# kanster/moped

Measured on AMD Instinct MI355X. Metric: detections/sec (frames/s) 640x480 ~3k SIFT vs N models, higher is better.
Workload: dtype f32

## Files before the change

include/moped_hip.h:

```cpp
#ifndef MOPED_HIP_H
#define MOPED_HIP_H

#include <stddef.h>
#include <stdint.h>

#ifdef __cplusplus
extern "C" {
#endif

#define MH_DESC_DIM 128
#define MH_MAX_BATCH 32
#define MH_MAX_IMAGES 8
#define MH_MAX_MODELS 8192
#define MH_OK 0
#define MH_ERR_ARG (-1)
#define MH_ERR_HIP (-2)
#define MH_ERR_CAPACITY (-3)
#define MH_ERR_NODEVICE (-4)

typedef struct mh_ctx mh_ctx;


int mh_create(int device, mh_ctx** out);
void mh_destroy(mh_ctx* ctx);
// ... 40 lines not shown
int mh_screen_values(mh_ctx* ctx, const float* q_host, int Q, int n_rows, float* out_host, float* dmax, float* spread,
                     int shape );
uint16_t mh_screen_record_value(float top, float thr);
void mh_screen_record_bounds(uint16_t value_bits, uint32_t row0, float tau, float spread, int N, float dmax, float* lo,
                             float* hi);
float mh_screen_pack_value(float v, uint32_t id, int bits);
float mh_screen_pack_pert(float qq, float dmax, int bits);
void mh_screen_sample_bounds(uint16_t value_bits, float tau, float pert, float dmax, float* lo, float* hi);
void mh_screen_launch_plan(int Q, int q_expected, int N, int32_t out[8]);
int mh_match_incomplete(mh_ctx* ctx, uint32_t* count, int reset);
int mh_screen_sample_values(mh_ctx* ctx, const float* q_host, int Q, const int32_t* row0_host, float* out_host);
int mh_match_query_candidates(mh_ctx* ctx, int Q, uint32_t* out);

int mh_match_local_dev(mh_ctx* ctx, const float* qn_dev, const float* qnorm_dev, int Q,
                       int32_t* idx1_dev, float* d1_dev, float* d2_dev);
int mh_match_merge_dev(mh_ctx* ctx, const int32_t* idx1_s_dev, const float* d1_s_dev,
                       const float* d2_s_dev, int n_shards, int Q,
                       int32_t* idx1_dev, float* d1_dev, float* d2_dev);
int mh_normalize_dev(mh_ctx* ctx, float* q_dev, float* qnorm_dev, int Q);


int mh_meanshift(mh_ctx* ctx, const float* pts_host, int n, int dim, float radius,
                 float merge, int min_pts, int max_iter, int32_t* label,
                 int32_t* order, int32_t* n_clusters);
int mh_meanshift_batch(mh_ctx* ctx, const float* pts_host, const int32_t* off, int n_problems,
                       int dim, float radius, float merge, int min_pts, int max_iter,
                       int32_t* label, int32_t* order, int32_t* n_clusters);


typedef struct {
// ... 304 lines not shown
```

moped_amd/capi.py:

```python
from __future__ import annotations

import ctypes as C
import os

import numpy as np

_HERE = os.path.dirname(os.path.abspath(__file__))
LIB_PATH = os.environ.get("MH_LIB_PATH") or os.path.join(_HERE, "libmoped_hip.so")

MH_OK = 0


class MhError(RuntimeError):
    pass


class mh_corr(C.Structure):
    _fields_ = [("u", C.c_float), ("v", C.c_float), ("x", C.c_float), ("y", C.c_float), ("z", C.c_float)]


class mh_cam(C.Structure):
    _fields_ = [("K", C.c_float * 4), ("cam", C.c_float * 7)]


# ... 50 lines not shown
        super().__init__(cutoff, min_pts, use3d_filter, sigma2d, sigma3d, linkage_type)


def default_linkage_params():
    return mh_linkage_params(0.1, 7, 2, -1.0, -1.0, 1)


class mh_depth_rules(C.Structure):
    _fields_ = [("patch_size", C.c_int32), ("feature_density", C.c_float), ("match_density", C.c_float),
                ("ratio_table", C.c_void_p), ("n_models", C.c_int32), ("maximum_depth", C.c_float),
                ("default_depth", C.c_float), ("cauchy_scale", C.c_float)]


EXPORTS = [
    "mh_create", "mh_destroy", "mh_last_error", "mh_set_stream", "mh_synchronize", "mh_reserve",
    "mh_db_upload", "mh_db_size", "mh_normalize", "mh_match", "mh_normalize_match", "mh_match_local_dev",
    "mh_match_merge_dev", "mh_normalize_dev", "mh_meanshift", "mh_meanshift_batch", "mh_pose_ransac", "mh_pose_ransac_depth",
    "mh_frame_set_depth", "mh_project_test",
    "mh_filter", "mh_frame_default_params", "mh_frame_enqueue", "mh_frame_set_depth_image", "mh_frame_enqueue_match_local",
    "mh_frame_enqueue_rest", "mh_frame_fetch", "mh_frame_result_dev", "mh_enable_timing", "mh_timing",
    "mh_frame_set_cluster_linkage", "mh_cluster_linkage", "mh_frame_set_depth_image_host",
    "mh_depth_fill", "mh_depth_fill_status", "mh_depth_fill_host",
    "mh_frame_enqueue_rest_batch", "mh_frame_enqueue_rest_frames", "mh_frame_fetch_slot", "mh_frame_result_copy_slots_dev",
    "mh_frame_set_depth_rules", "mh_frame_fetch_matches", "mh_frame_enqueue_rest_strided", "mh_frame_result_copy_dev",
    "mh_sift_extract", "mh_sift_extract_dev", "mh_frame_enqueue_image", "mh_frame_enqueue_image_batch", "mh_frame_features_dev", "mh_frame_keypoints",
    "mh_models_create", "mh_models_destroy", "mh_models_last_error", "mh_models_add_xml",
    "mh_models_add_xml_buffer", "mh_models_count", "mh_models_rows", "mh_models_name", "mh_models_range",
    "mh_models_desc", "mh_models_xyz", "mh_models_save", "mh_models_load", "mh_db_upload_models",
    "mh_db_splice", "mh_db_reserve", "mh_db_adopt", "mh_db_generation", "mh_db_model_rows", "mh_db_splice_models",
    "mh_db_debug_fetch", "mh_depth_rules_debug_fetch", "mh_db_debug_screen", "mh_db_debug_route", "mh_db_edit_ms",
    "mh_db_upload_raw", "mh_db_share", "mh_match_stats", "mh_match_set_mode", "mh_match_launches", "mh_pose_set_split", "mh_frame_fetch_match_points", "mh_screen_margin", "mh_frame_counters", "mh_match_timing", "mh_frame_set_images", "mh_filter_images",
# ... 43 lines not shown
    L.mh_last_error.restype = C.c_char_p
    L.mh_set_stream.argtypes = [vp, vp]
    L.mh_synchronize.argtypes = [vp]
    L.mh_reserve.argtypes = [vp, i32, i32, i32]
    L.mh_reserve_batch.argtypes = [vp, i32, i32, i32, i32]
    if hasattr(L, "mh_lane_create"):
        L.mh_lane_create.argtypes = [i32, i32, i32, i32, C.POINTER(vp)]
        L.mh_lane_destroy.argtypes = [vp]
        L.mh_set_lane.argtypes = [vp, vp]
    L.mh_db_upload.argtypes = [vp, vp, vp, vp, i32, i32, C.c_int32]
    L.mh_db_size.argtypes = [vp, C.POINTER(i32), C.POINTER(i32)]
    L.mh_normalize.argtypes = [vp, vp, i32]
    L.mh_match.argtypes = [vp, vp, i32, f32, vp, vp, vp, vp]
    L.mh_normalize_match.argtypes = [vp, vp, i32, f32, vp, vp, vp, vp]
    L.mh_match_local_dev.argtypes = [vp, vp, vp, i32, vp, vp, vp]
    L.mh_match_merge_dev.argtypes = [vp, vp, vp, vp, i32, i32, vp, vp, vp]
    L.mh_normalize_dev.argtypes = [vp, vp, vp, i32]
    L.mh_meanshift.argtypes = [vp, vp, i32, i32, f32, f32, i32, i32, vp, vp, C.POINTER(C.c_int32)]
    L.mh_meanshift_batch.argtypes = [vp, vp, vp, i32, i32, f32, f32, i32, i32, vp, vp, vp]
    L.mh_pose_ransac.argtypes = [vp, vp, vp, i32, C.POINTER(mh_cam), C.POINTER(mh_pose_params),
                                 C.c_uint64, vp, C.POINTER(C.c_int32)]
    L.mh_pose_ransac_depth.argtypes = [vp, vp, vp, vp, i32, C.POINTER(mh_cam), C.POINTER(mh_pose_params), i32, f32,
                                       C.c_uint64, vp, C.POINTER(C.c_int32)]
    L.mh_frame_set_depth.argtypes = [vp, vp, i32, f32]
    L.mh_project_test.argtypes = [vp, vp, vp, i32, C.POINTER(mh_cam), f32, vp, vp, C.POINTER(C.c_int32)]
    L.mh_filter.argtypes = [vp, vp, vp, i32, vp, vp, i32, C.POINTER(mh_cam), i32, f32, f32,
                            vp, vp, vp, vp, vp, C.POINTER(C.c_int32)]
    L.mh_frame_default_params.argtypes = [C.POINTER(mh_frame_params)]
    L.mh_frame_default_params.restype = None
    L.mh_frame_enqueue.argtypes = [vp, vp, vp, i32, C.POINTER(mh_cam), C.POINTER(mh_frame_params), C.c_uint64]
# ... 1172 lines not shown
        counts = np.zeros(4, np.int32)
        self._ck(self.L.mh_frame_fetch(self.h, _ptr(objs), max_objects, C.byref(n), _ptr(counts)), "mh_frame_fetch")
        return objs[:min(n.value, max_objects)].copy(), counts

    def frame_result_dev(self):
        p = C.c_void_p()
        b = C.c_int64(0)
        self._ck(self.L.mh_frame_result_dev(self.h, C.byref(p), C.byref(b)), "mh_frame_result_dev")
        return p.value, b.value

    def match_local_dev(self, qn_ptr, qnorm_ptr, Q, idx_ptr, d1_ptr, d2_ptr):
        self._ck(self.L.mh_match_local_dev(self.h, C.c_void_p(qn_ptr), C.c_void_p(qnorm_ptr), Q,
                                           C.c_void_p(idx_ptr), C.c_void_p(d1_ptr), C.c_void_p(d2_ptr)),
                 "mh_match_local_dev")

    def match_merge_dev(self, idx_s_ptr, d1_s_ptr, d2_s_ptr, n_shards, Q, idx_ptr, d1_ptr, d2_ptr):
        self._ck(self.L.mh_match_merge_dev(self.h, C.c_void_p(idx_s_ptr), C.c_void_p(d1_s_ptr),
                                           C.c_void_p(d2_s_ptr), n_shards, Q, C.c_void_p(idx_ptr),
                                           C.c_void_p(d1_ptr), C.c_void_p(d2_ptr)), "mh_match_merge_dev")

    def normalize_dev(self, q_ptr, qnorm_ptr, Q):
        self._ck(self.L.mh_normalize_dev(self.h, C.c_void_p(q_ptr), C.c_void_p(qnorm_ptr), Q), "mh_normalize_dev")


class ModelSet:

    def __init__(self, desc_type: str = "SIFT", _handle=None):
        self.L = load()
        if _handle is None:
            h = C.c_void_p()
# ... 84 lines not shown
```

moped_amd/csrc/api.hip:

```cpp
#include <algorithm>
#include <cmath>
#include <cstring>
#include <new>
#include <vector>

#include "context.h"
#include "steps.h"

using namespace mh;

namespace mh {

int use_stream(mh_ctx* ctx) {
  if (!ctx->held.empty()) db_poll_held(ctx, false);
  if (ctx->stream) return MH_OK;
  if (!ctx->own_stream) MH_HIP(ctx, hipStreamCreateWithFlags(&ctx->own_stream, hipStreamNonBlocking));
  ctx->stream = ctx->own_stream;
  return MH_OK;
}

int ensure_scratch(mh_ctx* ctx, size_t bytes) {
  if (bytes > ctx->scratch.cap) MH_HIP(ctx, ctx->scratch.ensure(bytes + bytes / 4 + 4096, ctx->stream));
  return MH_OK;
}
// ... 70 lines not shown
              const int32_t* q_count, int q_expected) {
  if (Q <= 0) return MH_OK;
  int rc = ensure_match_scratch(ctx, Q);
  if (rc) return rc;
  const int qe = (q_expected > 0 && q_expected < Q) ? q_expected : Q;
  const int screen_mode = ctx->match_mode >= 2 ? 0 : ctx->match_mode;
  const int kernel_pin = ctx->match_mode >= 2 ? ctx->match_mode - 2 : -1;
  if (ctx->sdb.usable && ctx->sbuf.q_pad >= screen_q_pad(Q) && screen_wanted(qe, ctx->N, screen_mode)) {
    ctx->sbuf.ev = nullptr;
    if (ctx->timing && ctx->ev_made) {
      ctx->sbuf.ev = ctx->mev[ctx->mev_next];
      ctx->mev_next = (ctx->mev_next + 1) % mh_ctx::MEV_SETS;
      ++ctx->mev_used;
    }
    ctx->sbuf.big = ctx->lane_stream;
    ctx->sbuf.ev_in = ctx->lane_in;
    ctx->sbuf.ev_out = ctx->lane_out;
    launch_match_screen(qn, qnorm, Q, ctx->db_desc, ctx->db_norm, ctx->N, ctx->rmap, ctx->sdb, ctx->sbuf, idx1, d1,
                        d2, ctx->stream, q_count, q_expected);
    ++ctx->match_launches[2];
  } else {
    const int k = launch_match(qn, qnorm, Q, ctx->db_desc, ctx->db_norm, ctx->N, ctx->rmap, ctx->match_scratch,
                               ctx->match_pack, idx1, d1, d2, ctx->stream, q_count, q_expected, kernel_pin);
    if (k >= 0) ++ctx->match_launches[k];
  }
  return MH_OK;
}

int ensure_frame_buffers(mh_ctx* ctx, int Q) {
  if (Q <= ctx->max_q) return MH_OK;
// ... 16 lines not shown
extern "C" {

int mh_create(int device, mh_ctx** out) {
  if (!out) return MH_ERR_ARG;
  *out = nullptr;
  int count = 0;
  if (hipGetDeviceCount(&count) != hipSuccess || count <= 0 || device < 0 || device >= count)
    return MH_ERR_NODEVICE;
  hipDeviceProp_t prop;
  if (hipGetDeviceProperties(&prop, device) != hipSuccess) return MH_ERR_NODEVICE;
  if (std::strncmp(prop.gcnArchName, "gfx950", 6) != 0) return MH_ERR_NODEVICE;
  if (hipSetDevice(device) != hipSuccess) return MH_ERR_HIP;
  mh_ctx* ctx = new (std::nothrow) mh_ctx;
  if (!ctx) return MH_ERR_HIP;
  ctx->device = device;
  ctx->stream = nullptr;
  *out = ctx;
  return MH_OK;
}

void mh_free_frame_state(mh_ctx* ctx);
void mh_free_sift_state(mh_ctx* ctx);
void mh_free_undistort_state(mh_ctx* ctx);

void mh_destroy(mh_ctx* ctx) {
  if (!ctx) return;
  hipSetDevice(ctx->device);
  if (ctx->stream) hipStreamSynchronize(ctx->stream);
  mh_free_frame_state(ctx);
  mh_free_sift_state(ctx);
// ... 273 lines not shown
}

int mh_match_local_dev(mh_ctx* ctx, const float* qn_dev, const float* qnorm_dev, int Q,
                       int32_t* idx1_dev, float* d1_dev, float* d2_dev) {
  if (!ctx || Q < 0 || (Q > 0 && (!qn_dev || !qnorm_dev || !idx1_dev || !d1_dev || !d2_dev)))
    return MH_ERR_ARG;
  if (Q == 0) return MH_OK;
  MH_HIP(ctx, hipSetDevice(ctx->device));
  if (int rc_stream = mh::use_stream(ctx)) return rc_stream;
  int rc = ctx_match(ctx, qn_dev, qnorm_dev, Q, idx1_dev, d1_dev, d2_dev);
  if (rc) return rc;
  MH_HIP(ctx, hipGetLastError());
  return MH_OK;
}

int mh_match_merge_dev(mh_ctx* ctx, const int32_t* idx1_s_dev, const float* d1_s_dev,
                       const float* d2_s_dev, int n_shards, int Q, int32_t* idx1_dev,
                       float* d1_dev, float* d2_dev) {
  if (!ctx || Q < 0 || n_shards < 0) return MH_ERR_ARG;
  if (Q == 0) return MH_OK;
  MH_HIP(ctx, hipSetDevice(ctx->device));
  if (int rc_stream = mh::use_stream(ctx)) return rc_stream;
  launch_match_merge(idx1_s_dev, d1_s_dev, d2_s_dev, n_shards, Q, (size_t)Q, idx1_dev, d1_dev, d2_dev,
                     ctx->stream);
  MH_HIP(ctx, hipGetLastError());
  return MH_OK;
}

static int match_host(mh_ctx* ctx, const float* q_host, float* normalized_out, int Q, float ratio, int32_t* nn_idx,
                      int32_t* nn_raw, float* d1, float* d2) {
// ... 280 lines not shown
```

moped_amd/csrc/context.h:

```cpp
#pragma once
#include <cmath>
#include <cstring>
#include <memory>
#include <mutex>
#include <string>
#include <vector>

#include "common.h"
#include "devbuf.h"
#include "screen.h"
#include "steps.h"

struct DbStore;

struct DbPool {
  std::mutex mu;
  size_t cap_rows = 0;
  int max_models = 0;
  DbStore* spare = nullptr;
  ~DbPool();
};

struct DbStore {
  int device = 0;
// ... 59 lines not shown
  st->screen.zero_idx = (int32_t)h[4];
  std::memcpy(&st->screen.zero_d1, &h[5], 4);
  std::memcpy(&st->screen.zero_d2, &h[6], 4);
  st->screen.usable = h[2] == 0 && x_max < 60000.f;
}

struct mh_lane {
  int device = 0;
  std::vector<hipStream_t> streams;
  unsigned next = 0;
  int reserve = 0, low_priority = 0;
};

struct mh_ctx {
  int device = 0;
  hipStream_t own_stream = nullptr;
  hipStream_t stream = nullptr;
  std::string err;

  std::shared_ptr<DbStore> store;
  int N = 0, n_models = 0;
  int32_t index_base = 0;
  mh::RowMap rmap;
  float* db_desc = nullptr;
  float* db_norm = nullptr;
  float* db_xyz = nullptr;
  int32_t* db_model = nullptr;
  mh::ScreenDb sdb;
  mh::ScreenBufs sbuf;
  struct ScreenOwn {
// ... 192 lines not shown
```

moped_amd/csrc/match_screen.hip:

```cpp
#include <hip/hip_fp16.h>

#include <algorithm>
#include <cstdlib>

#include "common.h"
#include "screen.h"

MH_TRACE_TU()

namespace mh {

namespace {

typedef _Float16 half8 __attribute__((ext_vector_type(8)));
typedef float v16f __attribute__((ext_vector_type(16)));
#define MH_AS1 __attribute__((address_space(1)))
#define MH_AS3 __attribute__((address_space(3)))

constexpr int SC_QPAD = 3 * 1024;
constexpr int SC_TILE = 128;
constexpr int SC_TILE_BYTES = SC_TILE * DIM * 2;
constexpr bool SC_SHAPE16_LARGE = true;
constexpr int SC_NW_LARGE = 8;
__host__ __device__ constexpr int sc_recbuf(int nw) { return nw >= 8 ? 112 : 40; }
// ... 963 lines not shown
  const float lose = better ? a.b1 : d;
  a.b2 = fminf(a.b2, lose);
  a.b1 = better ? d : a.b1;
  a.i1 = better ? row : a.i1;
}
__device__ __forceinline__ void merge(Best& a, float ob1, float ob2, int oi1) {
  const bool take_o = (ob1 < a.b1) || (ob1 == a.b1 && (unsigned)oi1 < (unsigned)a.i1);
  const float lose1 = take_o ? a.b1 : ob1;
  const float s2 = fminf(a.b2, ob2);
  a.b2 = fminf(lose1, s2);
  a.b1 = take_o ? ob1 : a.b1;
  a.i1 = take_o ? oi1 : a.i1;
}

constexpr int RS_WAVES = 4;
constexpr int RS_MAXC = 1024;
constexpr int RS_STAGE = 8;
static_assert(RS_STAGE * DIM * 4 <= RS_MAXC * 4 && RS_STAGE % 2 == 0 && RS_STAGE <= 32, "staged rows live in the candidate list's LDS");

__device__ __forceinline__ float exact_dist(const float* __restrict__ q_lds, const float* __restrict__ row, float nq, float dn) {
  float s = 0.f;
  const float4* r4 = reinterpret_cast<const float4*>(row);
#pragma unroll 2
  for (int c = 0; c < DIM / 16; ++c) {
    const float4 x0 = r4[4 * c], x1 = r4[4 * c + 1], x2 = r4[4 * c + 2], x3 = r4[4 * c + 3];
    const float4 y0 = *reinterpret_cast<const float4*>(q_lds + 16 * c), y1 = *reinterpret_cast<const float4*>(q_lds + 16 * c + 4);
    const float4 y2 = *reinterpret_cast<const float4*>(q_lds + 16 * c + 8), y3 = *reinterpret_cast<const float4*>(q_lds + 16 * c + 12);
    s = fmaf(y0.x, x0.x, s); s = fmaf(y0.y, x0.y, s); s = fmaf(y0.z, x0.z, s); s = fmaf(y0.w, x0.w, s);
    s = fmaf(y1.x, x1.x, s); s = fmaf(y1.y, x1.y, s); s = fmaf(y1.z, x1.z, s); s = fmaf(y1.w, x1.w, s);
    s = fmaf(y2.x, x2.x, s); s = fmaf(y2.y, x2.y, s); s = fmaf(y2.z, x2.z, s); s = fmaf(y2.w, x2.w, s);
// ... 18 lines not shown
  for (int s = 0; s < 4; ++s) a[s] = ap[4 * s];
  const int crow = (g < 2 ? row0x : row0y) + 16 * (g & 1);
  const float4 c = *reinterpret_cast<const float4*>(dneg + (size_t)(crow >> 7) * SC_DD + (crow & 127));
  v4f acc = {c.x, c.y, c.z, c.w};
#pragma unroll
  for (int s = 0; s < 4; ++s) {
    const float4 y0 = *reinterpret_cast<const float4*>(q_lds + 32 * s + 8 * g), y1 = *reinterpret_cast<const float4*>(q_lds + 32 * s + 8 * g + 4);
    half8 b;
    b[0] = (_Float16)y0.x; b[1] = (_Float16)y0.y; b[2] = (_Float16)y0.z; b[3] = (_Float16)y0.w;
    b[4] = (_Float16)y1.x; b[5] = (_Float16)y1.y; b[6] = (_Float16)y1.z; b[7] = (_Float16)y1.w;
    acc = __builtin_amdgcn_mfma_f32_16x16x32_f16(a[s], b, acc, 0, 0, 0);
  }
  return acc;
}

__global__ __launch_bounds__(64 * RS_WAVES) __attribute__((amdgpu_waves_per_eu(8, 8))) void rescore_kernel(
    const float* __restrict__ qn, const float* __restrict__ qnorm, const uint8_t* __restrict__ qbad, int Q,
    const int32_t* __restrict__ q_count, const float* __restrict__ db, const float* __restrict__ dnorm, int N,
    RowMap rmap, uint2* __restrict__ recs, int n_slots, int32_t* __restrict__ ovf_cnt, uint2* __restrict__ ovf,
    int ovf_cap, float dmax, const float* __restrict__ tau, float spread, int32_t* __restrict__ idx1, float* __restrict__ d1, float* __restrict__ d2,
    unsigned int* __restrict__ stats, int32_t zero_idx, float zero_d1, float zero_d2, SampleGeom g,
    const unsigned int* __restrict__ inc, unsigned int* __restrict__ inc_count, const _Float16* __restrict__ dbh,
    const float* __restrict__ dneg) {
  MH_TRACE_SCOPE(mh::TK_PASS_C);
  __shared__ __attribute__((aligned(16))) float q_s[RS_WAVES][DIM];
  __shared__ __attribute__((aligned(16))) int cand_s[RS_WAVES][RS_MAXC];
  __shared__ int ncand_s[RS_WAVES];
  __shared__ int samp_s[RS_WAVES][SC_SA_SLOTS];
  __shared__ int nsamp_s[RS_WAVES];
  const int lane = threadIdx.x & 63;
  const int wave = __builtin_amdgcn_readfirstlane(threadIdx.x >> 6);
  const int q = blockIdx.x * RS_WAVES + wave;
  if (q >= Q) return;
  constexpr int RS_ITERS = (SC_SLOT_PITCH + SCREEN_OVF_CAP + 63) / 64;
  uint2* mine = recs + (size_t)q * SC_SLOT_PITCH;
  const int n_own = n_slots + g.sa_slots;
  auto slot_at = [&](int j) -> uint2& { return mine[j < n_slots ? j : SC_SLOTS_MAX + (j - n_slots)]; };
  uint2 recv[RS_ITERS];
#pragma unroll
  for (int it = 0; it < RS_ITERS; ++it) {
    const int j = it * 64 + lane;
    recv[it] = j < n_own ? slot_at(j) : make_uint2(0u, 0u);
  }
  const int Qe = q_count ? min(Q, *q_count) : Q;
  const int bad = qbad[q];
  const float nq = qnorm[q];
  const float tau_q = tau[q];
  const int n_ovf = ovf_cnt[q];
  const unsigned incw = inc ? inc[q] : 0u;
  const float2 qv = reinterpret_cast<const float2*>(qn + (size_t)q * DIM)[lane];
  asm volatile("" ::"v"(bad), "v"(nq), "v"(tau_q), "v"(n_ovf), "v"(incw), "v"(qv.x), "v"(qv.y), "s"(Qe));
  if (q >= Qe) {
    if (lane == 0) {
      idx1[q] = -1;
      d1[q] = __builtin_inff();
      d2[q] = __builtin_inff();
    }
    return;
  }
  if (bad == 2) {
    if (lane == 0) {
      idx1[q] = -1;
      d1[q] = __builtin_inff();
      d2[q] = __builtin_inff();
    }
    return;
  }
  if (bad == 3) {
    if (lane == 0) {
      idx1[q] = zero_idx >= 0 ? row_to_global(rmap, zero_idx) : -1;
      d1[q] = zero_d1;
      d2[q] = zero_d2;
      if (stats) stats[3 * q + 2] += 1u;
    }
    return;
  }
  if (lane == 0) {
    ncand_s[wave] = 0;
    nsamp_s[wave] = 0;
  }
  q_s[wave][2 * lane] = qv.x;
  q_s[wave][2 * lane + 1] = qv.y;
  bool brute = n_ovf > ovf_cap || bad == 1;
  int n_cand = 0;
  if (!brute) {
    float l1 = -__builtin_inff(), l2 = -__builtin_inff();
    const float pert = screen_pack_pert(nq, dmax, g.pack_bits);
    auto bounds = [tau_q, spread, N, dmax, pert](uint2 rec, float& lo, float& hi) {
      if (rec.x & SC_REC_SAMPLE) screen_sample_bounds((unsigned short)(rec.y >> 16), tau_q, pert, dmax, lo, hi);
      else screen_record_bounds((unsigned short)(rec.y >> 16), rec.x & 0x3FFFFFFFu, tau_q, spread, N, dmax, lo, hi);
    };
#pragma unroll
    for (int it = 0; it < RS_ITERS; ++it) {
      const int j = it * 64 + lane;
      uint2 rec = recv[it];
      if (j < n_own) {
        if (rec.y) slot_at(j) = make_uint2(0u, 0u);
// ... 15 lines not shown
      l1 = fmaxf(l1, o1);
    }
    const float keep_from = l2 - screen_margin(nq, dmax);
#pragma unroll
    for (int it = 0; it < RS_ITERS; ++it) {
      const uint2 rec = recv[it];
      unsigned bits = rec.y & 0xFFFFu;
      if (bits) {
        float lo, hi;
        bounds(rec, lo, hi);
        if (hi < keep_from) bits = 0;
      }
      const int hi_stride = (rec.x & 0x80000000u) ? 16 : 8;
      const int row0 = (int)(rec.x & 0x3FFFFFFFu);
      if (bits && (rec.x & SC_REC_SAMPLE)) {
        const int w = atomicAdd(&nsamp_s[wave], 1);
        if (w < SC_SA_SLOTS) samp_s[wave][w] = row0;
        bits = 0;
      }
      while (bits) {
        const int r = __builtin_ctz(bits);
        bits &= bits - 1;
        const int w = atomicAdd(&ncand_s[wave], 1);
        if (w < RS_MAXC) cand_s[wave][w] = row0 + (r & 3) + hi_stride * (r >> 2);
      }
    }
    wave_lds_sync();
    const int n_samp = min(nsamp_s[wave], SC_SA_SLOTS), n_pad_rows = (N + SC_TILE - 1) / SC_TILE * SC_TILE;
    for (int p = 0; p < n_samp; p += 2) {
      const bool pair = p + 1 < n_samp;
      const int rx = samp_s[wave][p], ry = samp_s[wave][pair ? p + 1 : p];
      if (rx + 19 >= n_pad_rows || ry + 19 >= n_pad_rows) continue;
      const v4f w = sample_pair_values(q_s[wave], dbh, dneg, rx, ry, lane);
      const int grp = lane >> 4;
      if ((lane & 15) == 0 && (grp < 2 || pair)) {
        const int base = (grp < 2 ? rx : ry) + 16 * (grp & 1);
#pragma unroll
        for (int r = 0; r < 4; ++r)
          if (w[r] > tau_q) {
            const int at = atomicAdd(&ncand_s[wave], 1);
            if (at < RS_MAXC) cand_s[wave][at] = base + r;
          }
      }
    }
    if (n_samp) wave_lds_sync();
    n_cand = ncand_s[wave];
    if (n_cand > RS_MAXC) brute = true;
  } else if (n_ovf > ovf_cap) {
    for (int j = lane; j < n_own; j += 64) slot_at(j) = make_uint2(0u, 0u);
  }
  if (n_ovf && lane == 0) ovf_cnt[q] = 0;
  wave_lds_sync();

  Best best = {__builtin_inff(), __builtin_inff(), -1};
  const int n_rows = brute ? N : n_cand;
  if (!brute && n_cand <= 64) {
    const int my_row = lane < n_cand ? cand_s[wave][lane] : -1;
    const bool my_ok = my_row >= 0 && my_row < N;
    const float my_dn = my_ok ? dnorm[my_row] : 0.f;
    wave_lds_sync();
    float4* stage = reinterpret_cast<float4*>(cand_s[wave]);
    const int n_st = min(n_cand, RS_STAGE);
    const int half = lane >> 5, c = lane & 31;
    float4 v[RS_STAGE / 2];
#pragma unroll
    for (int i = 0; i < RS_STAGE / 2; ++i) {
      const int r = 2 * i + half;
      const int row_r = __shfl(my_row, r);
      v[i] = make_float4(0.f, 0.f, 0.f, 0.f);
      if (r < n_st && row_r >= 0 && row_r < N) v[i] = reinterpret_cast<const float4*>(db + (size_t)row_r * DIM)[c];
    }
#pragma unroll
    for (int i = 0; i < RS_STAGE / 2; ++i) {
      const int r = 2 * i + half;
      if (r < n_st) stage[r * 32 + (c ^ r)] = v[i];
    }
    wave_lds_sync();
    if (lane < n_st) {
      if (my_ok) {
        float sdot = 0.f;
        const float4* qs4 = reinterpret_cast<const float4*>(q_s[wave]);
#pragma unroll 8
        for (int k = 0; k < 32; ++k) {
          const float4 x = stage[lane * 32 + (k ^ lane)], y = qs4[k];
          sdot = fmaf(y.x, x.x, sdot); sdot = fmaf(y.y, x.y, sdot); sdot = fmaf(y.z, x.z, sdot); sdot = fmaf(y.w, x.w, sdot);
        }
        take(best, fmaxf(fmaf(-2.f, sdot, nq + my_dn), 0.f), my_row);
      }
    } else if (my_ok) {
      take(best, exact_dist(q_s[wave], db + (size_t)my_row * DIM, nq, my_dn), my_row);
    }
  } else {
    for (int k = lane; k < n_rows; k += 64) {
      const int row = brute ? k : cand_s[wave][k];
      if (row >= 0 && row < N) take(best, exact_dist(q_s[wave], db + (size_t)row * DIM, nq, dnorm[row]), row);
    }
  }
  if (incw && !brute) {
    for (unsigned sm = incw & 0x0FFFFFFFu; sm; sm &= sm - 1) {
      const int split = __builtin_ctz(sm);
      const int sel0 = split * g.tiles_base + min(split, g.tiles_rem);
      const int sel1 = min(sel0 + g.tiles_base + (split < g.tiles_rem ? 1 : 0), g.n_sel);
      for (int k = sel0 * SC_TILE + lane; k < sel1 * SC_TILE; k += 64) {
        const int row = (g.tile_first + (k >> 7) * g.tile_stride) * SC_TILE + (k & 127);
        if (((incw >> (28 + ((k & 15) >> 2))) & 1u) && row < N)
          take(best, exact_dist(q_s[wave], db + (size_t)row * DIM, nq, dnorm[row]), row);
      }
    }
    if (lane == 0 && inc_count) atomicAdd(inc_count, 1u);
  }
#pragma unroll
  for (int d = 1; d < 64; d <<= 1) {
    const float ob1 = __shfl_xor(best.b1, d), ob2 = __shfl_xor(best.b2, d);
    const int oi1 = __shfl_xor(best.i1, d);
    if (oi1 >= 0) merge(best, ob1, ob2, oi1);
  }
  if (lane == 0) {
    idx1[q] = best.i1 >= 0 ? row_to_global(rmap, best.i1) : -1;
    d1[q] = best.b1;
    d2[q] = best.b2;
    if (stats) {
      stats[3 * q] += (unsigned)n_cand;
      stats[3 * q + 1] += brute ? 1u : 0u;
      stats[3 * q + 2] += 1u;
    }
  }
}

__global__ __launch_bounds__(64) void screen_values_kernel(const _Float16* __restrict__ qh, const _Float16* __restrict__ dbh,
                                                           const float* __restrict__ dneg, int n_rows, float* __restrict__ out,
                                                           int shape16) {
  const int lane = threadIdx.x, half = lane >> 5, l32 = lane & 31;
  const int q0 = blockIdx.x * 32, r0 = blockIdx.y * 32;
  if (shape16) {
    const int quarter = lane >> 4, l16 = lane & 15;
#pragma unroll
    for (int ti = 0; ti < 2; ++ti)
#pragma unroll
      for (int tj = 0; tj < 2; ++tj) {
        v4f acc;
#pragma unroll
        for (int r = 0; r < 4; ++r) {
// ... 253 lines not shown
  a.n_sel = p.n_sel_b;
  a.tile_first = 0;
  a.tile_stride = 1;
  a.skip_first = p.onesweep ? p.tile_first : 0;
  a.skip_stride = p.onesweep ? p.stride : 0;
  a.n_splits = p.Sb;
  a.tiles_base = p.n_sel_b / p.Sb;
  a.tiles_rem = p.n_sel_b % p.Sb;
  a.sub_cap = p.sub_cap;
  hipLaunchKernelGGL((screen16_kernel<1, NQB>), dim3(nqb * p.Sb), dim3(512), SC_LDS16_BYTES, s, a);
  if (ev) hipEventRecord(ev[4], s);
  *n_slots_out = 4 * p.Sb * a.sub_cap;
  *geom_out = g;
}

struct ShapeChoice {
  int nqb_sel;
  bool passes16;
};
ShapeChoice choose_shape(int qe, int n_tiles) {
  static const int nqb_pin = exp_int("MH_SCREEN_NQB", 0);
  int nqb_sel = qe > 640 ? 2 : 1;
  if (qe >= 2048 && (long)n_tiles * ((qe + 1023) / 1024) >= 16L * 256) nqb_sel = 4;
  if (nqb_pin >= 1 && nqb_pin <= 4) nqb_sel = nqb_pin;
  static const int shape_pin = exp_int("MH_SCREEN_SHAPE", 0);
  const bool shape16 = shape_pin == 2 || (shape_pin == 0 && SC_SHAPE16_LARGE);
  const bool p16 = shape16 && ((nqb_sel == 4 && (shape_pin == 2 || (qe + 1023) / 1024 >= 12)) || (nqb_sel == 2 && shape_pin == 2));
  return {nqb_sel, p16};
}

// ... 68 lines not shown
  SampleGeom geom = {0, 0, 0, 1, 0, 0, 0};
  static const int nw_pin = exp_int("MH_SCREEN_NW", 0);
  const int nw_sel = nw_pin == 4 || nw_pin == 8 ? nw_pin : (nqb_sel == 4 ? SC_NW_LARGE : 8);
  if (shape.passes16 && nqb_sel == 4) launch_passes16<4>(a, Q, qe, n_tiles, sample, blocks_a, blocks_b, &n_slots, &geom, sb.inc, sb.ev, sbig);
  else if (shape.passes16) launch_passes16<2>(a, Q, qe, n_tiles, sample, blocks_a, blocks_b, &n_slots, &geom, sb.inc, sb.ev, sbig);
  else if (nqb_sel == 4 && nw_sel == 4) launch_passes<4, 4>(a, Q, qe, n_tiles, sample, blocks_a, blocks_b, &n_slots, sb.ev, sbig, 256);
  else if (nqb_sel == 4) launch_passes<4, 8>(a, Q, qe, n_tiles, sample, blocks_a, blocks_b, &n_slots, sb.ev, sbig, 256);
  else if (nqb_sel == 3) launch_passes<3, 8>(a, Q, qe, n_tiles, sample, blocks_a, blocks_b, &n_slots, sb.ev, sbig, 256);
  else if (nqb_sel == 2 && nw_sel == 4) launch_passes<2, 4>(a, Q, qe, n_tiles, sample, blocks_a, blocks_b, &n_slots, sb.ev, sbig, 256);
  else if (nqb_sel == 2) launch_passes<2, 8>(a, Q, qe, n_tiles, sample, blocks_a, blocks_b, &n_slots, sb.ev, sbig, 256);
  else launch_passes<1, 8>(a, Q, qe, n_tiles, sample, blocks_a, blocks_b, &n_slots, sb.ev, sbig, 256);
  if (sbig != s) {
    hipEventRecord(sb.ev_out, sbig);
    hipStreamWaitEvent(s, sb.ev_out, 0);
  }
  hipLaunchKernelGGL(rescore_kernel, dim3((Q + RS_WAVES - 1) / RS_WAVES), dim3(64 * RS_WAVES), 0, s, qn, qnorm, sb.qbad, Q,
                     q_count, db, dnorm, N, rmap, sb.recs, n_slots, sb.ovf_cnt, sb.ovf, sb.ovf_cap, sdb.dmax, (const float*)sb.tau, sdb.spread, idx1, d1, d2,
                     sb.stats, sdb.zero_idx, sdb.zero_d1, sdb.zero_d2, geom, geom.sa_slots > 0 ? (const unsigned int*)sb.inc : nullptr,
                     sb.inc ? sb.inc + sb.q_pad : nullptr, sdb.dbh, sdb.dneg);
  if (sb.ev) hipEventRecord(sb.ev[5], s);
}

}
```

moped_amd/csrc/screen.h:

```cpp
#pragma once
#include <hip/hip_fp16.h>
#include <hip/hip_runtime.h>
#include <stdint.h>

namespace mh {

struct ScreenDb {
  const _Float16* dbh = nullptr;
  const float* dneg = nullptr;
  float dmax = 0.f;
  float spread = __builtin_inff();
  bool usable = false;
  int32_t zero_idx = -1;
  float zero_d1 = __builtin_inff(), zero_d2 = __builtin_inff();
};

struct ScreenBufs {
  _Float16* qh = nullptr;
  uint8_t* qbad = nullptr;
  float2* part = nullptr;
  float* tau = nullptr;
  uint2* recs = nullptr;
  int32_t* ovf_cnt = nullptr;
  uint2* ovf = nullptr;
  int ovf_cap = 0, q_pad = 0;
  hipEvent_t* ev = nullptr;
  hipStream_t big = nullptr;
  hipEvent_t ev_in = nullptr, ev_out = nullptr;
  unsigned int* stats = nullptr;
  unsigned int* inc = nullptr;
};

__host__ __device__ inline unsigned short screen_record_value(float top, float thr) {
  const _Float16 h = (_Float16)(top - thr);
  unsigned short b;
  __builtin_memcpy(&b, &h, 2);
  return b;
}
__host__ __device__ inline void screen_record_bounds(unsigned short value_bits, unsigned row0, float tau_q, float spread, int N,
                                                     float dmax, float& lo, float& hi) {
  _Float16 h;
  __builtin_memcpy(&h, &value_bits, 2);
  const float dv = (float)h;
  const float eps = fabsf(dv) * 0.001f + 1e-6f + 4e-7f * (fabsf(tau_q) + 0.5f * dmax * dmax);
  const bool fin = fabsf(dv) < 6.0e4f && fabsf(tau_q) < 1e30f;
// ... 52 lines not shown
```

Baseline: 16390.

## Restructure rescore kernel into persistent templated form with optional prefetch

The rescore (pass C) kernel now takes a single argument struct read from the kernarg segment, uses dynamic LDS, and loops over queries with a grid stride. It can prefetch the next query's slot records and scalars. Fat-block and prefetch variants sit behind an experiment flag, so the default path still launches the 4-wave, non-prefetch variant with one query per wave. The change also adds a counted-match API entry point and records the CU count. The default path keeps the same work but changes how arguments are loaded and adds dynamic LDS, which may shift register pressure.

```diff
diff --git a/include/moped_hip.h b/include/moped_hip.h
--- a/include/moped_hip.h
+++ b/include/moped_hip.h
@@ -78,6 +78,9 @@
 
 int mh_match_local_dev(mh_ctx* ctx, const float* qn_dev, const float* qnorm_dev, int Q,
                        int32_t* idx1_dev, float* d1_dev, float* d2_dev);
+int mh_match_local_counted_dev(mh_ctx* ctx, const float* qn_dev, const float* qnorm_dev, int Q,
+                               const int32_t* q_count_dev, int q_expected, int32_t* idx1_dev, float* d1_dev,
+                               float* d2_dev);
 int mh_match_merge_dev(mh_ctx* ctx, const int32_t* idx1_s_dev, const float* d1_s_dev,
                        const float* d2_s_dev, int n_shards, int Q,
                        int32_t* idx1_dev, float* d1_dev, float* d2_dev);
diff --git a/moped_amd/capi.py b/moped_amd/capi.py
--- a/moped_amd/capi.py
+++ b/moped_amd/capi.py
@@ -88,7 +88,7 @@
 
 EXPORTS = [
     "mh_create", "mh_destroy", "mh_last_error", "mh_set_stream", "mh_synchronize", "mh_reserve",
-    "mh_db_upload", "mh_db_size", "mh_normalize", "mh_match", "mh_normalize_match", "mh_match_local_dev",
+    "mh_db_upload", "mh_db_size", "mh_normalize", "mh_match", "mh_normalize_match", "mh_match_local_dev", "mh_match_local_counted_dev",
     "mh_match_merge_dev", "mh_normalize_dev", "mh_meanshift", "mh_meanshift_batch", "mh_pose_ransac", "mh_pose_ransac_depth",
     "mh_frame_set_depth", "mh_project_test",
     "mh_filter", "mh_frame_default_params", "mh_frame_enqueue", "mh_frame_set_depth_image", "mh_frame_enqueue_match_local",
@@ -162,6 +162,8 @@
     L.mh_match.argtypes = [vp, vp, i32, f32, vp, vp, vp, vp]
     L.mh_normalize_match.argtypes = [vp, vp, i32, f32, vp, vp, vp, vp]
     L.mh_match_local_dev.argtypes = [vp, vp, vp, i32, vp, vp, vp]
+    if hasattr(L, "mh_match_local_counted_dev"):
+        L.mh_match_local_counted_dev.argtypes = [vp, vp, vp, i32, vp, i32, vp, vp, vp]
     L.mh_match_merge_dev.argtypes = [vp, vp, vp, vp, i32, i32, vp, vp, vp]
     L.mh_normalize_dev.argtypes = [vp, vp, vp, i32]
     L.mh_meanshift.argtypes = [vp, vp, i32, i32, f32, f32, i32, i32, vp, vp, C.POINTER(C.c_int32)]
@@ -1364,6 +1366,11 @@
                                            C.c_void_p(idx_ptr), C.c_void_p(d1_ptr), C.c_void_p(d2_ptr)),
                  "mh_match_local_dev")
 
+    def match_local_counted_dev(self, qn_ptr, qnorm_ptr, Q, q_count_ptr, q_expected, idx_ptr, d1_ptr, d2_ptr):
+        self._ck(self.L.mh_match_local_counted_dev(self.h, C.c_void_p(qn_ptr), C.c_void_p(qnorm_ptr), Q, C.c_void_p(q_count_ptr),
+                                                   int(q_expected), C.c_void_p(idx_ptr), C.c_void_p(d1_ptr), C.c_void_p(d2_ptr)),
+                 "mh_match_local_counted_dev")
+
     def match_merge_dev(self, idx_s_ptr, d1_s_ptr, d2_s_ptr, n_shards, Q, idx_ptr, d1_ptr, d2_ptr):
         self._ck(self.L.mh_match_merge_dev(self.h, C.c_void_p(idx_s_ptr), C.c_void_p(d1_s_ptr),
                                            C.c_void_p(d2_s_ptr), n_shards, Q, C.c_void_p(idx_ptr),
diff --git a/moped_amd/csrc/api.hip b/moped_amd/csrc/api.hip
--- a/moped_amd/csrc/api.hip
+++ b/moped_amd/csrc/api.hip
@@ -108,6 +108,7 @@
       ++ctx->mev_used;
     }
     ctx->sbuf.big = ctx->lane_stream;
+    ctx->sbuf.n_cus = ctx->n_cus;
     ctx->sbuf.ev_in = ctx->lane_in;
     ctx->sbuf.ev_out = ctx->lane_out;
     launch_match_screen(qn, qnorm, Q, ctx->db_desc, ctx->db_norm, ctx->N, ctx->rmap, ctx->sdb, ctx->sbuf, idx1, d1,
@@ -154,6 +155,7 @@
   mh_ctx* ctx = new (std::nothrow) mh_ctx;
   if (!ctx) return MH_ERR_HIP;
   ctx->device = device;
+  ctx->n_cus = prop.multiProcessorCount;
   ctx->stream = nullptr;
   *out = ctx;
   return MH_OK;
@@ -457,6 +459,19 @@
   return MH_OK;
 }
 
+int mh_match_local_counted_dev(mh_ctx* ctx, const float* qn_dev, const float* qnorm_dev, int Q, const int32_t* q_count_dev,
+                               int q_expected, int32_t* idx1_dev, float* d1_dev, float* d2_dev) {
+  if (!ctx || Q < 0 || q_expected < 0 || !q_count_dev || (Q > 0 && (!qn_dev || !qnorm_dev || !idx1_dev || !d1_dev || !d2_dev)))
+    return MH_ERR_ARG;
+  if (Q == 0) return MH_OK;
+  MH_HIP(ctx, hipSetDevice(ctx->device));
+  if (int rc_stream = mh::use_stream(ctx)) return rc_stream;
+  int rc = ctx_match(ctx, qn_dev, qnorm_dev, Q, idx1_dev, d1_dev, d2_dev, q_count_dev, q_expected);
+  if (rc) return rc;
+  MH_HIP(ctx, hipGetLastError());
+  return MH_OK;
+}
+
 int mh_match_merge_dev(mh_ctx* ctx, const int32_t* idx1_s_dev, const float* d1_s_dev,
                        const float* d2_s_dev, int n_shards, int Q, int32_t* idx1_dev,
                        float* d1_dev, float* d2_dev) {
diff --git a/moped_amd/csrc/context.h b/moped_amd/csrc/context.h
--- a/moped_amd/csrc/context.h
+++ b/moped_amd/csrc/context.h
@@ -97,6 +97,7 @@
 
 struct mh_ctx {
   int device = 0;
+  int n_cus = 0;
   hipStream_t own_stream = nullptr;
   hipStream_t stream = nullptr;
   std::string err;
diff --git a/moped_amd/csrc/match_screen.hip b/moped_amd/csrc/match_screen.hip
--- a/moped_amd/csrc/match_screen.hip
+++ b/moped_amd/csrc/match_screen.hip
@@ -1,3 +1,4 @@
+#include <type_traits>
 #include <hip/hip_fp16.h>
 
 #include <algorithm>
@@ -1001,6 +1002,10 @@
 }
 
 constexpr int RS_WAVES = 4;
+#ifdef MH_EXPERIMENTS
+constexpr int RS_WAVES_FAT = 16;
+constexpr int RS_FAT_K = 2;
+#endif
 constexpr int RS_MAXC = 1024;
 constexpr int RS_STAGE = 8;
 static_assert(RS_STAGE * DIM * 4 <= RS_MAXC * 4 && RS_STAGE % 2 == 0 && RS_STAGE <= 32, "staged rows live in the candidate list's LDS");
@@ -1049,41 +1054,92 @@
   return acc;
 }
 
-__global__ __launch_bounds__(64 * RS_WAVES) __attribute__((amdgpu_waves_per_eu(8, 8))) void rescore_kernel(
-    const float* __restrict__ qn, const float* __restrict__ qnorm, const uint8_t* __restrict__ qbad, int Q,
-    const int32_t* __restrict__ q_count, const float* __restrict__ db, const float* __restrict__ dnorm, int N,
+constexpr int RS_ITERS = (SC_SLOT_PITCH + SCREEN_OVF_CAP + 63) / 64;
+struct RsScalars {
+  int bad;
+  float nq, tau_q;
+  int n_ovf;
+  unsigned incw;
+  float2 qv;
+};
+constexpr size_t rs_lds_bytes(int waves) { return (size_t)waves * (DIM * 4 + RS_MAXC * 4 + SC_SA_SLOTS * 4 + 8); }
+
+struct RsArgs {
+  const float* qn;
+  const float* qnorm;
+  const uint8_t* qbad;
+  int Q;
+  const int32_t* q_count;
+  const float* db;
+  const float* dnorm;
+  int N;
+  RowMap rmap;
+  uint2* recs;
+  int n_slots;
+  int32_t* ovf_cnt;
+  uint2* ovf;
+  int ovf_cap;
+  float dmax;
+  const float* tau;
+  float spread;
+  int32_t* idx1;
+  float* d1;
+  float* d2;
+  unsigned int* stats;
+  int32_t zero_idx;
+  float zero_d1, zero_d2;
+  SampleGeom g;
+  const unsigned int* inc;
+  unsigned int* inc_count;
+  const _Float16* dbh;
+  const float* dneg;
+};
+typedef const __attribute__((address_space(4))) RsArgs* RsArgsPtr;
+__device__ __forceinline__ RsArgsPtr rs_args() {
+  RsArgsPtr p = (RsArgsPtr)__builtin_amdgcn_kernarg_segment_ptr();
+  asm volatile("" : "+s"(p));
+  return p;
+}
+
+__device__ __forceinline__ void rs_load_slots(const uint2* recs, int n_slots, int sa_slots, int q, int lane, uint2 (&rv)[RS_ITERS]) {
+  const uint2* theirs = recs + (size_t)q * SC_SLOT_PITCH;
+  const int n_own = n_slots + sa_slots;
+#pragma unroll
+  for (int it = 0; it < RS_ITERS; ++it) {
+    const int j = it * 64 + lane;
+    rv[it] = j < n_own ? theirs[j < n_slots ? j : SC_SLOTS_MAX + (j - n_slots)] : make_uint2(0u, 0u);
+  }
+}
+#define RS_CONST(T, p) ((const __attribute__((address_space(4))) T*)(p))
+__device__ __forceinline__ RsScalars rs_load_scalars(const uint8_t* qbad, const float* qnorm, const float* tau, const int32_t* ovf_cnt,
+                                                     const unsigned int* inc, const float* qn, int q, int lane) {
+  RsScalars v;
+  v.qv = reinterpret_cast<const float2*>(qn + (size_t)q * DIM)[lane];
+  v.n_ovf = RS_CONST(int32_t, ovf_cnt)[q];
+  const unsigned w = RS_CONST(unsigned int, inc ? inc : reinterpret_cast<const unsigned int*>(tau))[q];
+  v.bad = (RS_CONST(unsigned int, qbad)[q >> 2] >> (8 * (q & 3))) & 0xFFu;
+  v.nq = RS_CONST(float, qnorm)[q];
+  v.tau_q = RS_CONST(float, tau)[q];
+  v.incw = inc ? w : 0u;
+  return v;
+}
+
+__device__ __forceinline__ void rescore_query(
+    int q, int lane, float* q_sw, int* cand_sw, int* samp_sw, int* ncand_sw, int* nsamp_sw, uint2 (&recv)[RS_ITERS], const RsScalars sc, int Qe,
+    const float* __restrict__ db, const float* __restrict__ dnorm, int N,
     RowMap rmap, uint2* __restrict__ recs, int n_slots, int32_t* __restrict__ ovf_cnt, uint2* __restrict__ ovf,
-    int ovf_cap, float dmax, const float* __restrict__ tau, float spread, int32_t* __restrict__ idx1, float* __restrict__ d1, float* __restrict__ d2,
+    int ovf_cap, float dmax, float spread, int32_t* __restrict__ idx1, float* __restrict__ d1, float* __restrict__ d2,
     unsigned int* __restrict__ stats, int32_t zero_idx, float zero_d1, float zero_d2, SampleGeom g,
-    const unsigned int* __restrict__ inc, unsigned int* __restrict__ inc_count, const _Float16* __restrict__ dbh,
-    const float* __restrict__ dneg) {
-  MH_TRACE_SCOPE(mh::TK_PASS_C);
-  __shared__ __attribute__((aligned(16))) float q_s[RS_WAVES][DIM];
-  __shared__ __attribute__((aligned(16))) int cand_s[RS_WAVES][RS_MAXC];
-  __shared__ int ncand_s[RS_WAVES];
-  __shared__ int samp_s[RS_WAVES][SC_SA_SLOTS];
-  __shared__ int nsamp_s[RS_WAVES];
-  const int lane = threadIdx.x & 63;
-  const int wave = __builtin_amdgcn_readfirstlane(threadIdx.x >> 6);
-  const int q = blockIdx.x * RS_WAVES + wave;
-  if (q >= Q) return;
-  constexpr int RS_ITERS = (SC_SLOT_PITCH + SCREEN_OVF_CAP + 63) / 64;
+    unsigned int* __restrict__ inc_count, const _Float16* __restrict__ dbh, const float* __restrict__ dneg) {
   uint2* mine = recs + (size_t)q * SC_SLOT_PITCH;
   const int n_own = n_slots + g.sa_slots;
   auto slot_at = [&](int j) -> uint2& { return mine[j < n_slots ? j : SC_SLOTS_MAX + (j - n_slots)]; };
-  uint2 recv[RS_ITERS];
-#pragma unroll
-  for (int it = 0; it < RS_ITERS; ++it) {
-    const int j = it * 64 + lane;
-    recv[it] = j < n_own ? slot_at(j) : make_uint2(0u, 0u);
-  }
-  const int Qe = q_count ? min(Q, *q_count) : Q;
-  const int bad = qbad[q];
-  const float nq = qnorm[q];
-  const float tau_q = tau[q];
-  const int n_ovf = ovf_cnt[q];
-  const unsigned incw = inc ? inc[q] : 0u;
-  const float2 qv = reinterpret_cast<const float2*>(qn + (size_t)q * DIM)[lane];
+  const int bad = sc.bad;
+  const float nq = sc.nq;
+  const float tau_q = sc.tau_q;
+  const int n_ovf = sc.n_ovf;
+  const unsigned incw = sc.incw;
+  const float2 qv = sc.qv;
   asm volatile("" ::"v"(bad), "v"(nq), "v"(tau_q), "v"(n_ovf), "v"(incw), "v"(qv.x), "v"(qv.y), "s"(Qe));
   if (q >= Qe) {
     if (lane == 0) {
@@ -1110,12 +1166,13 @@
     }
     return;
   }
+  wave_lds_sync();
   if (lane == 0) {
-    ncand_s[wave] = 0;
-    nsamp_s[wave] = 0;
-  }
-  q_s[wave][2 * lane] = qv.x;
-  q_s[wave][2 * lane + 1] = qv.y;
+    *ncand_sw = 0;
+    *nsamp_sw = 0;
+  }
+  q_sw[2 * lane] = qv.x;
+  q_sw[2 * lane + 1] = qv.y;
   bool brute = n_ovf > ovf_cap || bad == 1;
   int n_cand = 0;
   if (!brute) {
@@ -1161,37 +1218,37 @@
       const int hi_stride = (rec.x & 0x80000000u) ? 16 : 8;
       const int row0 = (int)(rec.x & 0x3FFFFFFFu);
       if (bits && (rec.x & SC_REC_SAMPLE)) {
-        const int w = atomicAdd(&nsamp_s[wave], 1);
-        if (w < SC_SA_SLOTS) samp_s[wave][w] = row0;
+        const int w = atomicAdd(nsamp_sw, 1);
+        if (w < SC_SA_SLOTS) samp_sw[w] = row0;
         bits = 0;
       }
       while (bits) {
         const int r = __builtin_ctz(bits);
         bits &= bits - 1;
-        const int w = atomicAdd(&ncand_s[wave], 1);
-        if (w < RS_MAXC) cand_s[wave][w] = row0 + (r & 3) + hi_stride * (r >> 2);
+        const int w = atomicAdd(ncand_sw, 1);
+        if (w < RS_MAXC) cand_sw[w] = row0 + (r & 3) + hi_stride * (r >> 2);
       }
     }
     wave_lds_sync();
-    const int n_samp = min(nsamp_s[wave], SC_SA_SLOTS), n_pad_rows = (N + SC_TILE - 1) / SC_TILE * SC_TILE;
+    const int n_samp = min(*nsamp_sw, SC_SA_SLOTS), n_pad_rows = (N + SC_TILE - 1) / SC_TILE * SC_TILE;
     for (int p = 0; p < n_samp; p += 2) {
       const bool pair = p + 1 < n_samp;
-      const int rx = samp_s[wave][p], ry = samp_s[wave][pair ? p + 1 : p];
+      const int rx = samp_sw[p], ry = samp_sw[pair ? p + 1 : p];
       if (rx + 19 >= n_pad_rows || ry + 19 >= n_pad_rows) continue;
-      const v4f w = sample_pair_values(q_s[wave], dbh, dneg, rx, ry, lane);
+      const v4f w = sample_pair_values(q_sw, dbh, dneg, rx, ry, lane);
       const int grp = lane >> 4;
       if ((lane & 15) == 0 && (grp < 2 || pair)) {
         const int base = (grp < 2 ? rx : ry) + 16 * (grp & 1);
 #pragma unroll
         for (int r = 0; r < 4; ++r)
           if (w[r] > tau_q) {
-            const int at = atomicAdd(&ncand_s[wave], 1);
-            if (at < RS_MAXC) cand_s[wave][at] = base + r;
+            const int at = atomicAdd(ncand_sw, 1);
+            if (at < RS_MAXC) cand_sw[at] = base + r;
           }
       }
     }
     if (n_samp) wave_lds_sync();
-    n_cand = ncand_s[wave];
+    n_cand = *ncand_sw;
     if (n_cand > RS_MAXC) brute = true;
   } else if (n_ovf > ovf_cap) {
     for (int j = lane; j < n_own; j += 64) slot_at(j) = make_uint2(0u, 0u);
@@ -1202,11 +1259,11 @@
   Best best = {__builtin_inff(), __builtin_inff(), -1};
   const int n_rows = brute ? N : n_cand;
   if (!brute && n_cand <= 64) {
-    const int my_row = lane < n_cand ? cand_s[wave][lane] : -1;
+    const int my_row = lane < n_cand ? cand_sw[lane] : -1;
     const bool my_ok = my_row >= 0 && my_row < N;
     const float my_dn = my_ok ? dnorm[my_row] : 0.f;
     wave_lds_sync();
-    float4* stage = reinterpret_cast<float4*>(cand_s[wave]);
+    float4* stage = reinterpret_cast<float4*>(cand_sw);
     const int n_st = min(n_cand, RS_STAGE);
     const int half = lane >> 5, c = lane & 31;
     float4 v[RS_STAGE / 2];
@@ -1226,7 +1283,7 @@
     if (lane < n_st) {
       if (my_ok) {
         float sdot = 0.f;
-        const float4* qs4 = reinterpret_cast<const float4*>(q_s[wave]);
+        const float4* qs4 = reinterpret_cast<const float4*>(q_sw);
 #pragma unroll 8
         for (int k = 0; k < 32; ++k) {
           const float4 x = stage[lane * 32 + (k ^ lane)], y = qs4[k];
@@ -1235,12 +1292,12 @@
         take(best, fmaxf(fmaf(-2.f, sdot, nq + my_dn), 0.f), my_row);
       }
     } else if (my_ok) {
-      take(best, exact_dist(q_s[wave], db + (size_t)my_row * DIM, nq, my_dn), my_row);
+      take(best, exact_dist(q_sw, db + (size_t)my_row * DIM, nq, my_dn), my_row);
     }
   } else {
     for (int k = lane; k < n_rows; k += 64) {
-      const int row = brute ? k : cand_s[wave][k];
-      if (row >= 0 && row < N) take(best, exact_dist(q_s[wave], db + (size_t)row * DIM, nq, dnorm[row]), row);
+      const int row = brute ? k : cand_sw[k];
+      if (row >= 0 && row < N) take(best, exact_dist(q_sw, db + (size_t)row * DIM, nq, dnorm[row]), row);
     }
   }
   if (incw && !brute) {
@@ -1251,7 +1308,7 @@
       for (int k = sel0 * SC_TILE + lane; k < sel1 * SC_TILE; k += 64) {
         const int row = (g.tile_first + (k >> 7) * g.tile_stride) * SC_TILE + (k & 127);
         if (((incw >> (28 + ((k & 15) >> 2))) & 1u) && row < N)
-          take(best, exact_dist(q_s[wave], db + (size_t)row * DIM, nq, dnorm[row]), row);
+          take(best, exact_dist(q_sw, db + (size_t)row * DIM, nq, dnorm[row]), row);
       }
     }
     if (lane == 0 && inc_count) atomicAdd(inc_count, 1u);
@@ -1273,6 +1330,56 @@
     }
   }
 }
+
+template <int WAVES, int PF>
+__global__ __launch_bounds__(64 * WAVES) __attribute__((amdgpu_waves_per_eu(WAVES == 12 ? 6 : 8, WAVES == 12 ? 6 : 8))) void rescore_kernel(const RsArgs args) {
+  MH_TRACE_SCOPE(mh::TK_PASS_C);
+  extern __shared__ __attribute__((aligned(16))) unsigned char rs_lds[];
+  const int lane0 = threadIdx.x & 63;
+  const int wave0 = __builtin_amdgcn_readfirstlane(threadIdx.x >> 6);
+  const int q_first = blockIdx.x * WAVES + wave0, q_stride = (int)gridDim.x * WAVES;
+  if (q_first >= args.Q) return;
+  const int Qe = args.q_count ? min(args.Q, *RS_CONST(int32_t, args.q_count)) : args.Q;
+  uint2 recv_next[RS_ITERS];
+  RsScalars sc_next = {};
+  if (PF >= 1) rs_load_slots(args.recs, args.n_slots, args.g.sa_slots, q_first, lane0, recv_next);
+  if (PF >= 2) sc_next = rs_load_scalars(args.qbad, args.qnorm, args.tau, args.ovf_cnt, args.inc, args.qn, q_first, lane0);
+  for (int q = q_first;; q += q_stride) {
+    int lane = lane0, wave = wave0;
+    asm volatile("" : "+v"(lane), "+s"(wave));
+    float* const q_sw = reinterpret_cast<float*>(rs_lds) + wave * DIM;
+    int* const cand_sw = reinterpret_cast<int*>(rs_lds + (size_t)WAVES * DIM * 4) + wave * RS_MAXC;
+    int* const samp_sw = reinterpret_cast<int*>(rs_lds + (size_t)WAVES * (DIM + RS_MAXC) * 4) + wave * SC_SA_SLOTS;
+    int* const ncand_sw = reinterpret_cast<int*>(rs_lds + (size_t)WAVES * (DIM + RS_MAXC + SC_SA_SLOTS) * 4) + wave;
+    int* const nsamp_sw = ncand_sw + WAVES;
+    const RsArgsPtr A = rs_args();
+    const int Q = A->Q;
+    if (q >= Q) break;
+    uint2 recv[RS_ITERS];
+    if (PF >= 1) {
+#pragma unroll
+      for (int it = 0; it < RS_ITERS; ++it) recv[it] = recv_next[it];
+    } else {
+      rs_load_slots(A->recs, A->n_slots, A->g.sa_slots, q, lane, recv);
+    }
+    const RsScalars sc = PF >= 2 ? sc_next : rs_load_scalars(A->qbad, A->qnorm, A->tau, A->ovf_cnt, A->inc, A->qn, q, lane);
+    if (PF >= 1 && q + q_stride < Q) {
+      rs_load_slots(A->recs, A->n_slots, A->g.sa_slots, q + q_stride, lane, recv_next);
+      if (PF >= 2) sc_next = rs_load_scalars(A->qbad, A->qnorm, A->tau, A->ovf_cnt, A->inc, A->qn, q + q_stride, lane);
+    }
+    RowMap rmap;
+    rmap.glo = A->rmap.glo;
+    rmap.llo = A->rmap.llo;
+    rmap.nb = A->rmap.nb;
+    rmap.base = A->rmap.base;
+    const SampleGeom g = {A->g.sa_slots, A->g.pack_bits, A->g.tile_first, A->g.tile_stride, A->g.tiles_base, A->g.tiles_rem, A->g.n_sel};
+    rescore_query(q, lane, q_sw, cand_sw, samp_sw, ncand_sw, nsamp_sw, recv, sc, Qe, A->db, A->dnorm, A->N, rmap, A->recs,
+                  A->n_slots, A->ovf_cnt, A->ovf, A->ovf_cap, A->dmax, A->spread, A->idx1, A->d1, A->d2, A->stats, A->zero_idx,
+                  A->zero_d1, A->zero_d2, g, A->inc_count, A->dbh, A->dneg);
+  }
+}
+static_assert(std::is_same<decltype(&rescore_kernel<RS_WAVES, 0>), void (*)(RsArgs)>::value,
+              "rs_args() reads RsArgs from offset 0 of the kernel argument segment: it must stay the only parameter");
 
 __global__ __launch_bounds__(64) void screen_values_kernel(const _Float16* __restrict__ qh, const _Float16* __restrict__ dbh,
                                                            const float* __restrict__ dneg, int n_rows, float* __restrict__ out,
@@ -1556,6 +1663,13 @@
   *geom_out = g;
 }
 
+template <int WAVES, int PF>
+void launch_pass_c(int grid, hipStream_t s, const RsArgs& args) {
+  static DynLds attr;
+  attr.ensure(rescore_kernel<WAVES, PF>, rs_lds_bytes(WAVES));
+  hipLaunchKernelGGL((rescore_kernel<WAVES, PF>), dim3(grid), dim3(64 * WAVES), rs_lds_bytes(WAVES), s, args);
+}
+
 struct ShapeChoice {
   int nqb_sel;
   bool passes16;
@@ -1654,10 +1768,28 @@
     hipEventRecord(sb.ev_out, sbig);
     hipStreamWaitEvent(s, sb.ev_out, 0);
   }
-  hipLaunchKernelGGL(rescore_kernel, dim3((Q + RS_WAVES - 1) / RS_WAVES), dim3(64 * RS_WAVES), 0, s, qn, qnorm, sb.qbad, Q,
-                     q_count, db, dnorm, N, rmap, sb.recs, n_slots, sb.ovf_cnt, sb.ovf, sb.ovf_cap, sdb.dmax, (const float*)sb.tau, sdb.spread, idx1, d1, d2,
-                     sb.stats, sdb.zero_idx, sdb.zero_d1, sdb.zero_d2, geom, geom.sa_slots > 0 ? (const unsigned int*)sb.inc : nullptr,
-                     sb.inc ? sb.inc + sb.q_pad : nullptr, sdb.dbh, sdb.dneg);
+  RsArgs ca;
+  ca.qn = qn; ca.qnorm = qnorm; ca.qbad = sb.qbad; ca.Q = Q; ca.q_count = q_count; ca.db = db; ca.dnorm = dnorm; ca.N = N;
+  ca.rmap = rmap; ca.recs = sb.recs; ca.n_slots = n_slots; ca.ovf_cnt = sb.ovf_cnt; ca.ovf = sb.ovf; ca.ovf_cap = sb.ovf_cap;
+  ca.dmax = sdb.dmax; ca.tau = sb.tau; ca.spread = sdb.spread; ca.idx1 = idx1; ca.d1 = d1; ca.d2 = d2; ca.stats = sb.stats;
+  ca.zero_idx = sdb.zero_idx; ca.zero_d1 = sdb.zero_d1; ca.zero_d2 = sdb.zero_d2; ca.g = geom;
+  ca.inc = geom.sa_slots > 0 ? sb.inc : nullptr; ca.inc_count = sb.inc ? sb.inc + sb.q_pad : nullptr; ca.dbh = sdb.dbh; ca.dneg = sdb.dneg;
+#ifdef MH_EXPERIMENTS
+  static const int pc_waves = exp_int("MH_PASSC_WAVES", RS_WAVES), pc_k = exp_int("MH_PASSC_K", RS_FAT_K);
+  static const int pc_pf = exp_int("MH_PASSC_PREFETCH", 0), pc_all = exp_int("MH_PASSC_FAT_ALL", 0);
+  const int n_cus = sb.n_cus > 0 ? sb.n_cus : 256;
+  const int fat_waves = pc_waves == 12 ? 12 : RS_WAVES_FAT;
+  if (pc_waves != RS_WAVES && (pc_all || Q > RS_FAT_K * n_cus * RS_WAVES_FAT)) {
+    const int cover = (Q + fat_waves - 1) / fat_waves, grid = pc_k > 0 ? std::min(cover, pc_k * n_cus) : cover;
+    if (fat_waves == 12 && pc_pf == 0) launch_pass_c<12, 0>(grid, s, ca);
+    else if (fat_waves == 12 && pc_pf == 1) launch_pass_c<12, 1>(grid, s, ca);
+    else if (fat_waves == 12) launch_pass_c<12, 2>(grid, s, ca);
+    else if (pc_pf == 0) launch_pass_c<RS_WAVES_FAT, 0>(grid, s, ca);
+    else if (pc_pf == 1) launch_pass_c<RS_WAVES_FAT, 1>(grid, s, ca);
+    else launch_pass_c<RS_WAVES_FAT, 2>(grid, s, ca);
+  } else
+#endif
+  launch_pass_c<RS_WAVES, 0>((Q + RS_WAVES - 1) / RS_WAVES, s, ca);
   if (sb.ev) hipEventRecord(sb.ev[5], s);
 }
 
diff --git a/moped_amd/csrc/screen.h b/moped_amd/csrc/screen.h
--- a/moped_amd/csrc/screen.h
+++ b/moped_amd/csrc/screen.h
@@ -29,6 +29,7 @@
   hipEvent_t ev_in = nullptr, ev_out = nullptr;
   unsigned int* stats = nullptr;
   unsigned int* inc = nullptr;
+  int n_cus = 0;
 };
 
 __host__ __device__ inline unsigned short screen_record_value(float top, float thr) {
```

New measurement: 16630 (median of 6 runs). 1.4% higher.
